# sevagh/Zen

Hardware: AMD Instinct MI355X
Metric: hops/sec (1024-hop HPR, 44.1 kHz mono) (higher is better)
Workload: dtype f32

## Files before the change

zen_amd/csrc/fft_dev.h:

```cpp
#pragma once
#include <type_traits>
#include <hip/hip_runtime.h>

#pragma clang fp contract(off)

namespace zfft {

template <int V>
struct Log2 {
	static constexpr int value = 1 + Log2<V / 2>::value;
};
template <>
struct Log2<1> {
	static constexpr int value = 0;
};

#ifndef ZEN_FFT16K_V
#define ZEN_FFT16K_V 16
#endif

template <int LOG2N>
struct Plan {
	static_assert(LOG2N >= 5 && LOG2N <= 14, "nfft 32..16384");
	static_assert(ZEN_FFT16K_V == 16 || ZEN_FFT16K_V == 32, "16 or 32 values per thread");
// ... 350 lines not shown
			}
		}
#ifdef ZEN_FFT_INPLACE
		if ((FIRST && SYNC_FIRST) || (!FIRST && (!INPL || LAST)))
			frame_sync<TF>();
#else
		if (!FIRST || SYNC_FIRST)
			frame_sync<TF>();
#endif
#pragma unroll
		for (int i = 0; i < NB; ++i) {
			const int b = tf + i * TF;
			const int k = b >> log2J;
			if constexpr (PRE)
				butterfly<R, INV, ZUP, (FIRST && TW::PLAIN)>(v[i], k, sL, LOG2N, twp, PASS, i);
			else
				butterfly<R, INV, ZUP, (FIRST && TW::PLAIN)>(v[i], k, sL, LOG2N, tw, PASS, i);
#pragma unroll
			for (int c = 0; c < R; ++c) {
				const int idx = b + c * (N / R);
				if (LAST) {
					if (!HALF_OUT || c < R / 2) {
						if (active)
							out(idx, v[i][c], c < R / 2, c * NB + i);
					}
				}
#ifdef ZEN_FFT_INPLACE
				else if constexpr (INPL) {
					lds[PL::pad((image_k(k) * R + c) * J + (b & (J - 1)))] = v[i][c];
				}
#endif
				else {
#ifdef ZEN_FFT_FOLD_ADDR
					lds[PL::pad_off(b, c * (N / R))] = v[i][c];
#else
					lds[PL::pad(idx)] = v[i][c];
#endif
				}
			}
		}
		if constexpr (!LAST) {
			frame_sync<TF>();
			PassRunner<LOG2N, PASS + 1, INV, ZU, HALF_OUT, In, Out, SYNC_FIRST, TW>::run(tf, lds, tw, in, out, active);
		}
	}
};

template <int LOG2N, bool INV, bool ZU, bool HALF_OUT, class In, class Out, bool SYNC_FIRST = false>
__device__ __forceinline__ void fft_frame(int tf, float2* __restrict__ lds, const float2* __restrict__ tw,
                                          In& in, Out& out, bool active)
{
	const TwGlobal g{tw};
	PassRunner<LOG2N, 0, INV, ZU, HALF_OUT, In, Out, SYNC_FIRST, TwGlobal>::run(tf, lds, g, in, out, active);
}
template <int LOG2N, bool INV, bool ZU, bool HALF_OUT, class In, class Out, bool SYNC_FIRST = false>
__device__ __forceinline__ void fft_frame(int tf, float2* __restrict__ lds, const TwGlobalPre& tw, In& in, Out& out, bool active)
{
	PassRunner<LOG2N, 0, INV, ZU, HALF_OUT, In, Out, SYNC_FIRST, TwGlobalPre>::run(tf, lds, tw, in, out, active);
}
template <int LOG2N, bool INV, bool ZU, bool HALF_OUT, class In, class Out, bool SYNC_FIRST = false>
__device__ __forceinline__ void fft_frame(int tf, float2* __restrict__ lds, const TwLds& tw, In& in, Out& out, bool active)
{
	PassRunner<LOG2N, 0, INV, ZU, HALF_OUT, In, Out, SYNC_FIRST, TwLds>::run(tf, lds, tw, in, out, active);
}
template <int LOG2N, bool INV, bool ZU, bool HALF_OUT, class In, class Out, bool SYNC_FIRST = false>
__device__ __forceinline__ void fft_frame(int tf, float2* __restrict__ lds, const TwRegs<LOG2N>& tw, In& in, Out& out,
                                          bool active)
{
	PassRunner<LOG2N, 0, INV, ZU, HALF_OUT, In, Out, SYNC_FIRST, TwRegs<LOG2N>>::run(tf, lds, tw, in, out, active);
}

__device__ __forceinline__ double sqrt_of_sum_of_squares(double x)
{
	const double y = __builtin_amdgcn_rsq(x);
	double g = x * y;
	double h = 0.5 * y;
	const double r = __builtin_fma(-h, g, 0.5);
	g = __builtin_fma(g, r, g);
	h = __builtin_fma(h, r, h);
	double d = __builtin_fma(-g, g, x);
	g = __builtin_fma(d, h, g);
	d = __builtin_fma(-g, g, x);
	g = __builtin_fma(d, h, g);
	return (x == 0.0 || x == __builtin_inf()) ? x : g;
}

__device__ __forceinline__ float cabs_exact(float re, float im)
{
	const double r = (double)re, i = (double)im;
	return (float)sqrt_of_sum_of_squares(__builtin_fma(r, r, i * i));
}

}
```

zen_amd/csrc/hpr.hip:

```cpp
#include "common.h"
#include "memguard.h"
#include "filters.h"
#include "hpr_engine.h"
#include "host_pipe.h"

#include <algorithm>
#include <functional>
#include "sse_block.h"
#include "masks.h"
#include "rt_fused.h"
#include "stft.h"

#include <cfloat>
#include <climits>
#include <cmath>
#include <utility>
#include <vector>

using namespace zen_hip_impl;


namespace {
struct ProfScope {
	zen_hip_hpr* e;
// ... 175 lines not shown
	}
	e->tail_sel = 0;
	e->rows_stale = false;
	e->abs_frame = (long long)e->W - 1;
	e->last_frames = 0;
	e->drain[0] = e->drain[1] = e->drain[2] = 0;
	e->ready_valid[0] = e->ready_valid[1] = e->ready_valid[2] = false;
	if (e->d_wide_bar) {
		ZH_HIP(hipStreamSynchronize(e->stream));
		ZH_HIP(hipMemset2DAsync(e->d_wide_bar + 1, sizeof(unsigned) * 4, 0, sizeof(unsigned), S, e->stream));
		*e->wide_fail_host = 0;
	}
	return ZEN_HIP_OK;
}

int ensure_estimates(zen_hip_hpr* e, bool need_h)
{
	const size_t bytes = sizeof(float) * e->n_streams * e->max_hops * e->nfft;
	if (!e->d_P) {
		ZH_HIP(zh_malloc((void**)&e->d_P, bytes));
		ZH_HIP(hipMemsetAsync(e->d_P, 0, bytes, e->stream));
	}
	if (need_h && !e->d_H) {
		ZH_HIP(zh_malloc((void**)&e->d_H, bytes));
		ZH_HIP(hipMemsetAsync(e->d_H, 0, bytes, e->stream));
	}
	return ZEN_HIP_OK;
}

int ensure_rows(zen_hip_hpr* e, int o)
{
	if (e->d_Y[o])
		return ZEN_HIP_OK;
	const size_t bytes = sizeof(float) * e->n_streams * e->max_hops * e->nwin;
	ZH_HIP(zh_malloc((void**)&e->d_Y[o], bytes));
	ZH_HIP(hipMemsetAsync(e->d_Y[o], 0, bytes, e->stream));
	return ZEN_HIP_OK;
}

enum HopKernel { HOP_FUSED = 0, HOP_SSE = 1, HOP_WIDE = 2 };

void fused_args(zen_hip_hpr* e, const float* in, size_t in_stride, size_t M, RtFusedArgs& a)
{
	memset(&a, 0, sizeof(a));
	a.in = in;
	a.in_stride = (long long)in_stride;
	a.tail_prev = e->d_tail[e->tail_sel];
	a.tail_next = e->d_tail[e->tail_sel ^ 1];
	a.window = e->d_window;
	a.tw = e->d_tw;
	a.S = M == 1 ? e->d_S : nullptr;
	a.s_stride = (long long)e->s_stride;
	a.mag = e->d_mag;
	a.keep_mag_rows = (int)e->W - 1;
	a.ring_rows = e->ring_rows;
	a.row0 = e->abs_frame;
	a.hop = (int)e->hop;
	a.n_frames = (int)M;
	a.n_streams = (int)e->n_streams;
	a.prev_frames = (int)e->last_frames;
	a.y_stream_stride = (long long)(e->max_hops * e->nwin);
	for (int o = 0; o < 3; ++o) {
		a.Y[o] = e->d_Y[o];
		e->ready_valid[o] = false;
		if (output_computed(e, o)) {
			a.carry[o] = e->d_carry[o];
			a.out_id[a.n_out++] = o;
			a.ready[o] = e->ready_dev[o];
			e->ready_valid[o] = (M == 1);
		}
	}
	if (M == 1)
		a.seq = ++e->hop_seq;
	a.publish_seq = e->ready_host[0] != nullptr ? (g_opt_publish_release ? 2 : 1) : 0;
	a.beta = e->beta;
	a.beta_h = e->beta - FLT_EPSILON;
	a.cola = e->cola;
	a.soft = e->soft ? 1 : 0;
	a.power = (int)e->beta;
	a.out_h = e->out_h ? 1 : 0;
	a.out_p = e->out_p ? 1 : 0;
	a.thr = ZH_DIAG_OPT(g_opt_mask_divide) ? 0.0 : hard_mask_threshold(e->beta, &a.thr_inclusive);
	a.thr_h = ZH_DIAG_OPT(g_opt_mask_divide) ? 0.0 : hard_mask_threshold(a.beta_h, &a.thr_h_inclusive);
	a.diag = ZH_DIAG_OPT(g_opt_rt_fused_diag);
	a.stamps = e->dbg_stamps;
}

int wide_args(zen_hip_hpr* e, RtFusedArgs& a, hipStream_t stream, bool clear_votes = true)
{
	ZH_TRY(ensure_estimates(e, false));
	if (!e->d_wide_xch) {
		ZH_HIP(zh_malloc((void**)&e->d_wide_xch, sizeof(float2) * e->n_streams * e->nfft));
		ZH_HIP(zh_malloc((void**)&e->d_wide_bar, sizeof(unsigned) * 4 * e->n_streams + 16));
		ZH_HIP(hipMemsetAsync(e->d_wide_bar, 0, sizeof(unsigned) * 4 * e->n_streams + 16, e->stream));
		e->wide_arrivals = 0;
		e->wide_calls = 0;
		void* dev = nullptr;
		ZH_HIP(zh_host_malloc((void**)&e->wide_fail_host, 64, hipHostMallocMapped | hipHostMallocPortable));
		*e->wide_fail_host = 0;
		ZH_HIP(zh_host_device_pointer(&dev, e->wide_fail_host));
		e->wide_fail_dev = (unsigned*)dev;
	}
	if (e->wide_votes_stale && clear_votes) {
		for (size_t st = 0; st < e->n_streams; ++st)
			ZH_HIP(hipMemsetAsync(e->d_wide_bar + 4 * st + 2, 0, 2 * sizeof(unsigned), stream));
		e->wide_votes_stale = false;
	}
	a.wide_fail = e->wide_fail_dev;
	a.P = e->d_P;
	a.p_stream_stride = (long long)(e->max_hops * e->nfft);
	a.xch = e->d_wide_xch;
	a.bar = e->d_wide_bar;
	a.bar_base = e->wide_arrivals;
	a.bar_parity = (int)(e->wide_calls++ & 1u);
	e->wide_arrivals += rt_wide_arrivals(e->log2n, a.n_out);
	return ZEN_HIP_OK;
}

int run_hop_fused(zen_hip_hpr* e, const float* in, size_t in_stride, size_t M, HopKernel kind = HOP_FUSED)
{
	const bool sse = kind == HOP_SSE;
	for (int o = 0; o < 3; ++o)
		if (output_computed(e, o))
			ZH_TRY(ensure_rows(e, o));
	RtFusedArgs a;
	fused_args(e, in, in_stride, M, a);
	if (kind == HOP_WIDE)
		ZH_TRY(wide_args(e, a, e->stream));
	int direct_o = -1;
	for (int o = 0; o < 3; ++o)
		e->direct_done[o] = false;
	bool all_dst = a.n_out > 0;
	for (int i = 0; i < a.n_out; ++i)
		all_dst = all_dst && e->direct_out[a.out_id[i]] != nullptr;
	if (kind == HOP_FUSED && all_dst && !g_opt_no_direct_out && rt_fused_direct_out_available(e->log2n, e->mf, a)) {
		direct_o = a.out_id[0];
		if (!e->d_blk_flag) {
			const size_t bytes = sizeof(unsigned) * e->n_streams * e->max_hops;
			ZH_HIP(zh_malloc((void**)&e->d_blk_flag, bytes));
			ZH_HIP(zh_malloc((void**)&e->d_blk_need, bytes));
			ZH_HIP(hipMemsetAsync(e->d_blk_flag, 0, bytes, e->stream));
			ZH_HIP(hipMemsetAsync(e->d_blk_need, 0, bytes, e->stream));
			e->blk_seq = 0;
		}
		for (int o = 0; o < 3; ++o)
			a.out_direct[o] = e->direct_out[o];
		a.out_direct_stride = e->direct_stride;
		a.direct_on = 1;
		a.blk_flag = e->d_blk_flag;
		a.blk_need = e->d_blk_need;
		e->blk_seq = (e->blk_seq + 1) & 0x0fffffffu;
		if (e->blk_seq == 0)
			e->blk_seq = 1;
		a.blk_seq = e->blk_seq;
	}
	{
		ProfScope ps(e, zen_hip_hpr::K_FUSED);
		if (kind == HOP_WIDE)
			ZH_TRY(launch_rt_wide(e->log2n, e->mf, a, e->stream));
		else if (sse)
			ZH_TRY(launch_rt_sse(e->log2n, a, e->mt, e->mf, (float)e->l_harm + 1.0F, (float)e->l_perc + 1.0F, e->stream));
		else
			ZH_TRY(launch_rt_fused(e->log2n, e->mf, a, e->stream));
	}
	if (direct_o >= 0) {
		ProfScope ps(e, zen_hip_hpr::K_FINALIZE);
// ... 1312 lines not shown
```

zen_amd/csrc/masks.h:

```cpp
#pragma once
#include <hip/hip_runtime.h>

#include <cfloat>
#include <cstring>

#pragma clang fp contract(off)

namespace zen_hip_impl {

struct MaskCfg {
	float beta, beta_h;
	int soft, power, sse, out_h, out_p;
};

__device__ __forceinline__ float powi(float x, int p)
{
	if (p <= 0)
		return 1.0F;
	float r = x;
	for (int i = 1; i < p; ++i)
		r = r * x;
	return r;
}

__device__ __forceinline__ float pmask_value(float h, float p, const MaskCfg& c)
{
	const float EPS = FLT_EPSILON;
	if (c.sse)
		return p * p / (p * p + h * h + EPS);
	if (c.soft) {
		const float xp = powi(p, c.power), yp = powi(h, c.power);
		return xp / (xp + yp + EPS);
	}
	return (float)((p / (h + EPS)) >= c.beta);
}

__device__ __forceinline__ float hmask_value(float h, float p, const MaskCfg& c)
{
	const float EPS = FLT_EPSILON;
	if (c.sse)
		return h * h / (h * h + p * p + EPS);
	if (c.soft) {
		const float xp = powi(h, c.power), yp = powi(p, c.power);
		return xp / (xp + yp + EPS);
	}
	return (float)((h / (p + EPS)) >= c.beta_h);
}

__device__ __forceinline__ float hard_mask_exact(float x, float d, double thr, bool  = false)
{
	const double t = thr * (double)d;
	return (double)x > t ? 1.0F : 0.0F;
}

__device__ __forceinline__ float mask_value(int which, float h, float p, const MaskCfg& c)
{
	if (which == 0)
		return pmask_value(h, p, c);
	if (which == 1)
		return hmask_value(h, p, c);
	const float hm = c.out_h ? hmask_value(h, p, c) : 0.0f;
	const float pm = c.out_p ? pmask_value(h, p, c) : 0.0f;
	return 1 - (hm + pm);
}

struct HardThr {
	double p, h;
	int p_inc, h_inc;
};

__device__ __forceinline__ float pmask_thr(float h, float p, const MaskCfg& c, const HardThr& t)
{
	if (!c.sse && !c.soft && t.p != 0.0)
		return hard_mask_exact(p, h + FLT_EPSILON, t.p, t.p_inc != 0);
	return pmask_value(h, p, c);
}
__device__ __forceinline__ float hmask_thr(float h, float p, const MaskCfg& c, const HardThr& t)
{
	if (!c.sse && !c.soft && t.h != 0.0)
		return hard_mask_exact(h, p + FLT_EPSILON, t.h, t.h_inc != 0);
	return hmask_value(h, p, c);
}
__device__ __forceinline__ float mask_value_thr(int which, float h, float p, const MaskCfg& c, const HardThr& t)
{
	if (which == 0)
		return pmask_thr(h, p, c, t);
	if (which == 1)
		return hmask_thr(h, p, c, t);
	const float hm = c.out_h ? hmask_thr(h, p, c, t) : 0.0f;
	const float pm = c.out_p ? pmask_thr(h, p, c, t) : 0.0f;
	return 1 - (hm + pm);
}

inline double hard_mask_threshold(float beta, int* inclusive)
{
	unsigned u;
	memcpy(&u, &beta, sizeof(u));
	const unsigned expo = (u >> 23) & 0xffu;
	if ((u >> 31) || expo == 0 || expo == 0xffu)
		return 0.0;
	const unsigned up = u - 1;
	float pred;
	memcpy(&pred, &up, sizeof(pred));
	*inclusive = 0;
	const double m = ((double)pred + (double)beta) * 0.5;
	return (u & 1u) == 0 ? m * (1.0 - 0x1p-50) : m;
}
inline HardThr hard_mask_thresholds(float beta, float beta_h, bool divide)
{
	HardThr t{0.0, 0.0, 0, 0};
	if (!divide) {
		t.p = hard_mask_threshold(beta, &t.p_inc);
		t.h = hard_mask_threshold(beta_h, &t.h_inc);
	}
	return t;
}

}
```

zen_amd/csrc/rt_fused.h:

```cpp
#pragma once
#include <hip/hip_runtime.h>

namespace zen_hip_impl {

struct RtFusedArgs {
	const float* in;
	long long in_stride;
	const float* tail_prev;
	float* tail_next;
	const float* window;
	const float2* tw;
	float2* S;
	long long s_stride;
	float* mag;
	int keep_mag_rows;
	long long ring_rows;
	long long row0;
	int hop;
	int n_frames;
	int n_streams;
	int prev_frames;
	float* carry[3];
	float* Y[3];
	long long y_stream_stride;
	float* ready[3];
	unsigned seq;
	int publish_seq;
	int n_out;
	int out_id[3];
	float beta, beta_h, cola;
	int soft, power, out_h, out_p;
	double thr;
	int thr_inclusive;
	double thr_h;
	int thr_h_inclusive;
	float* P;
	long long p_stream_stride;
	float2* xch;
	unsigned* bar;
	unsigned bar_base;
	int bar_parity;
	unsigned* wide_fail;
	float* out_direct[3];
	long long out_direct_stride;
	int direct_on;
	unsigned* blk_flag;
	unsigned* blk_need;
	unsigned blk_seq;
	int diag;
	unsigned long long* stamps;
};

struct ResidentCtl {
	unsigned seq;
	unsigned stop;
	unsigned long long pad;
};
struct ResidentOut {
	unsigned exited;
	unsigned last_seq;
	unsigned hops;
	unsigned pad;
};
int launch_rt_fused_resident(int log2n, int freq_len, const RtFusedArgs& a, const ResidentCtl* ctl, ResidentOut* ro, unsigned seq_start,
                             unsigned long long idle_ticks, unsigned max_hops, hipStream_t stream);
int launch_rt_sse_resident(int log2n, const RtFusedArgs& a, int len_t, int len_f, float fac_h, float fac_p, const ResidentCtl* ctl,
                           ResidentOut* ro, unsigned seq_start, unsigned long long idle_ticks, unsigned max_hops, hipStream_t stream);

#if defined(__HIPCC__)
struct HopOfArgs {
	static constexpr bool KEEP = false;
	const RtFusedArgs& a;
	__device__ __forceinline__ const float* in() const { return a.in; }
	__device__ __forceinline__ unsigned seq() const { return a.seq; }
	__device__ __forceinline__ long long row0() const { return a.row0; }
	__device__ __forceinline__ const float* tail_prev() const { return a.tail_prev; }
	__device__ __forceinline__ float* tail_next() const { return a.tail_next; }
	__device__ __forceinline__ int prev_frames() const { return a.prev_frames; }
};
struct HopVar {
	static constexpr bool KEEP = true;
	mutable float keep_prev[4], keep_carry[4];
	const float* in_;
	unsigned seq_;
	long long row0_;
	const float* tail_prev_;
	float* tail_next_;
	int prev_frames_;
	__device__ __forceinline__ const float* in() const { return in_; }
	__device__ __forceinline__ unsigned seq() const { return seq_; }
	__device__ __forceinline__ long long row0() const { return row0_; }
	__device__ __forceinline__ const float* tail_prev() const { return tail_prev_; }
	__device__ __forceinline__ float* tail_next() const { return tail_next_; }
	__device__ __forceinline__ int prev_frames() const { return prev_frames_; }
};

__device__ __forceinline__ bool resident_next_hop(const ResidentCtl* ctl, unsigned last, unsigned long long idle_ticks, bool leave,
                                                   unsigned* s_cmd, unsigned* sq_out)
{
	if (threadIdx.x == 0) {
		const unsigned long long t0 = __builtin_amdgcn_s_memrealtime();
		unsigned cmd = 2, sq = last;
		for (;;) {
			const unsigned long long w =
			    __hip_atomic_load(reinterpret_cast<const unsigned long long*>(&ctl->seq), __ATOMIC_RELAXED, __HIP_MEMORY_SCOPE_SYSTEM);
			sq = (unsigned)w;
			if (sq != last) {
				cmd = 1;
				break;
			}
			if ((unsigned)(w >> 32) != 0u)
				break;
			if (__builtin_amdgcn_s_memrealtime() - t0 > idle_ticks)
				break;
			__builtin_amdgcn_s_sleep(1);
		}
		s_cmd[0] = leave ? 2u : cmd;
		s_cmd[1] = sq;
// ... 44 lines not shown
```

zen_amd/csrc/rt_fused.hip:

```cpp
#include "common.h"
#include "fft_dev.h"
#include "masks.h"
#include "median47_core.h"
#include "median_net.h"
#include "rt_fused.h"

#include <type_traits>

#pragma clang fp contract(off)

namespace zen_hip_impl {
namespace {

using zfft::Plan;

inline bool hop_lat_takes(int log2n, const RtFusedArgs& a)
{
	return a.n_frames == 1 && log2n <= 12 && !g_opt_no_hop_lat && !a.diag;
}

template <int T>
struct RtImage {
	static constexpr int PAD = T >= 8 ? 4 : 0;
	static constexpr int STRIDE = T + PAD;
	static constexpr int LOG2T = T == 16 ? 4 : (T == 8 ? 3 : 2);
	static __device__ __forceinline__ int addr(int g) { return (g >> LOG2T) * STRIDE + (g & (T - 1)); }
	static constexpr int caddr(int g) { return (g / T) * STRIDE + (g % T); }
	static constexpr int words(int n) { return ((n + T - 1) / T) * STRIDE; }
};

struct Regs {
	float2 S[16];
	float mag[16];
};

template <int LOG2N>
struct FwdIn {
	const float* prev;
	const float* cur;
	const float* window;
	float* tail;
	int hop;
	__device__ __forceinline__ float2 operator()(int idx, int) const
	{
		ZH_CHK(idx < hop ? prev + idx : cur + (idx - hop), 1);
		ZH_CHK(window + idx, 1);
		const float x = idx < hop ? prev[idx] : cur[idx - hop];
		if (tail && idx >= hop) {
			ZH_CHK(tail + (idx - hop), 1);
			tail[idx - hop] = x;
		}
		return make_float2(x * window[idx], 0.0f);
	}
};

struct FwdInPre {
	float x[8], w[8];
	__device__ __forceinline__ float2 operator()(int, int slot) const { return make_float2(x[slot] * w[slot], 0.0f); }
};

template <int T, int TFN>
struct FwdOut {
	Regs* r;
	float2* S;
	float* mag;
	int* img;
	int n, mid_al;
	__device__ __forceinline__ void operator()(int idx, float2 X, bool lower, int slot) const
	{
		r->S[slot] = X;
		if (lower || idx == (n >> 1)) {
			const float m = zfft::cabs_exact(X.x, X.y);
			const int key = __float_as_int(m);
			const int mir = (idx == 0 || idx == (n >> 1)) ? idx : n - idx;
			static_assert(TFN % T == 0, "whole chunks per slot");
			constexpr int CH = (TFN / T) * RtImage<T>::STRIDE;
			const int tfl = idx - slot * TFN;
			const int a0 = RtImage<T>::addr(tfl + mid_al), a1 = RtImage<T>::addr(n - tfl + mid_al);
			img[a0 + slot * CH] = key;
			img[(idx == 0 || idx == (n >> 1)) ? a0 + slot * CH : a1 - slot * CH] = key;
			if (S) {
				ZH_CHK(S + idx, 1);
				S[idx] = X;
			}
			if (mag) {
				ZH_CHK(mag + idx, 1);
				ZH_CHK(mag + mir, 1);
				mag[idx] = m;
				mag[mir] = m;
			}
		}
	}
};

template <int N, int TF, int MID, bool HALF>
struct InvIn {
	const Regs* r;
	const float* P;
	MaskCfg cfg;
	int which;
	__device__ __forceinline__ float2 operator()(int idx, int slot) const
	{
		int pi = idx;
		if (HALF) {
			const int lo = slot * TF, hi = lo + TF - 1;
			if (hi <= N / 2)
				pi = idx;
			else if (lo > N / 2 && hi < N - MID)
				pi = N - idx;
			else
				pi = (idx > N / 2 && idx < N - MID) ? N - idx : idx;
		}
		const float2 z = r->S[slot];
		const float m = mask_value(which, r->mag[slot], P[pi], cfg);
		return make_float2(z.x * m, z.y * m);
	}
};

constexpr int LEAN_PC_WORD = 5184;
constexpr int LEAN_PC_TAIL = 2052;
constexpr int LEAN_EDGE_WORD = LEAN_PC_WORD + LEAN_PC_TAIL + 512 + 4;
template <int N, int TF, int MID, bool HARDP>
struct InvInLean {
	const Regs* r;
	const int* img;
	const float* pc;
	MaskCfg cfg;
	int which;
	double thr;
	bool thr_inclusive;
	__device__ __forceinline__ float2 operator()(int idx, int slot) const
	{
		const int lo = slot * TF, hi = lo + TF - 1;
		int pi;
		if (hi <= N / 2)
			pi = idx;
		else if (lo > N / 2 && hi < N - MID)
			pi = N - idx;
		else
			pi = (idx > N / 2 && idx < N - MID) ? N - idx : (idx > N / 2 ? idx - (N - 512) + LEAN_PC_TAIL : idx);
		const int g = idx + 24;
		const int g0 = g - slot * TF;
		const float mag = __int_as_float(img[(g0 >> 4) * 20 + (g0 & 15) + slot * (TF / 16) * 20]);
		const float2 z = r->S[slot];
		float m;
		if constexpr (HARDP)
			m = hard_mask_exact(pc[pi], mag + FLT_EPSILON, thr, thr_inclusive);
		else
			m = thr != 0.0 ? hard_mask_exact(pc[pi], mag + FLT_EPSILON, thr, thr_inclusive) : mask_value(which, mag, pc[pi], cfg);
		return make_float2(z.x * m, z.y * m);
	}
};

template <int N, int TF, int MID, bool HARDP>
__device__ __forceinline__ unsigned lean_mask_bits(const int* img, const float* pc, int tf, const MaskCfg& cfg, double thr_p,
                                                   double thr_h)
{
	unsigned bits = 0;
#pragma unroll
	for (int slot = 0; slot < 16; ++slot) {
		const int idx = tf + slot * TF, lo = slot * TF, hi = lo + TF - 1;
		int pi;
		if (hi <= N / 2)
			pi = idx;
		else if (lo > N / 2 && hi < N - MID)
			pi = N - idx;
		else
			pi = (idx > N / 2 && idx < N - MID) ? N - idx : (idx > N / 2 ? idx - (N - 512) + LEAN_PC_TAIL : idx);
		const int g = idx + 24;
		const int g0 = tf + 24;
		const float h = __int_as_float(img[(g0 >> 4) * 20 + (g0 & 15) + slot * (TF / 16) * 20]), p = pc[pi];
		(void)g;
		unsigned pm, hm;
		if constexpr (HARDP) {
			pm = cfg.out_p ? (unsigned)(hard_mask_exact(p, h + FLT_EPSILON, thr_p) != 0.0f) : 0u;
			hm = cfg.out_h ? (unsigned)(hard_mask_exact(h, p + FLT_EPSILON, thr_h) != 0.0f) : 0u;
		}
		else {
			const HardThr t{thr_p, thr_h, 0, 0};
			pm = cfg.out_p ? (unsigned)(pmask_thr(h, p, cfg, t) != 0.0f) : 0u;
			hm = cfg.out_h ? (unsigned)(hmask_thr(h, p, cfg, t) != 0.0f) : 0u;
		}
		bits |= (pm | (hm << 1)) << (2 * slot);
	}
	return bits;
}
struct InvInBits {
	const Regs* r;
	unsigned bits;
	int which;
	__device__ __forceinline__ float2 operator()(int, int slot) const
	{
		const float pm = (float)((bits >> (2 * slot)) & 1u), hm = (float)((bits >> (2 * slot + 1)) & 1u);
		const float m = which == 0 ? pm : (which == 1 ? hm : 1 - (hm + pm));
		const float2 z = r->S[slot];
		return make_float2(z.x * m, z.y * m);
	}
};

struct InvOut {
	float* Y;
	float cola;
	float* ready;
	const float* carry;
	int hop;
	__device__ __forceinline__ void operator()(int idx, float2 x, bool, int) const
	{
		const float y = x.x * cola;
		ZH_CHK(Y + idx, 1);
		Y[idx] = y;
		if (ready && idx < hop) {
			ZH_CHK(ready + idx, 1);
			ZH_CHK(carry + idx, 1);
			ready[idx] = carry[idx] + y;
		}
	}
};
__device__ __forceinline__ unsigned xcc_id_of_cu()
{
	unsigned v;
	asm volatile("s_getreg_b32 %0, hwreg(HW_REG_XCC_ID)" : "=s"(v));
	return v & 15u;
}
template <bool KEEP>
struct InvOutRegT {
	float* Y;
	float cola;
	float* ready;
	float cv[4];
	int hop;
	float* next;
	__device__ __forceinline__ void operator()(int idx, float2 x, bool, int slot) const
	{
		const float y = x.x * cola;
		ZH_CHK(Y + idx, 1);
		Y[idx] = y;
		if (ready && idx < hop) {
			ZH_CHK(ready + idx, 1);
			__hip_atomic_store(ready + idx, cv[slot & 3] + y, __ATOMIC_RELAXED, __HIP_MEMORY_SCOPE_SYSTEM);
		}
		if constexpr (KEEP) {
			if (slot >= 4)
				next[slot & 3] = y;
		}
	}
};
using InvOutReg = InvOutRegT<false>;

struct FwdInKeep {
	const float* prev;
	const float* cur;
	const float* window;
	float* next;
	int hop;
	__device__ __forceinline__ float2 operator()(int idx, int slot) const
	{
		float x;
		if (slot < 4) {
			x = prev[slot & 3];
		}
		else {
			ZH_CHK(cur + (idx - hop), 1);
			x = cur[idx - hop];
			next[slot & 3] = x;
		}
		ZH_CHK(window + idx, 1);
		return make_float2(x * window[idx], 0.0f);
	}
};

template <bool LIGHT = false>
__device__ __forceinline__ void publish_ready(unsigned* flag, unsigned seq, int tf, bool release = false)
{
	ZH_CHK(flag, 1);
	if (LIGHT && !release) {
		asm volatile("s_waitcnt vmcnt(0)" ::: "memory");
		__builtin_amdgcn_fence(__ATOMIC_RELEASE, "workgroup");
		__syncthreads();
		if (tf == 0)
			__hip_atomic_store(flag, seq, __ATOMIC_RELAXED, __HIP_MEMORY_SCOPE_SYSTEM);
	}
	else {
		__threadfence_system();
		__syncthreads();
		if (tf == 0)
			__hip_atomic_store(flag, seq, __ATOMIC_RELEASE, __HIP_MEMORY_SCOPE_SYSTEM);
	}
}

template <int LOG2N, int W, int MINB, bool SINGLE, bool LEAN = false, bool HARDP = false, class HV = HopOfArgs>
__device__ __forceinline__ void rt_fused_body(const RtFusedArgs& a, const unsigned bid, const HV& hv, const int tid)
{
	using PL = Plan<LOG2N>;
	constexpr int N = PL::N, TF = PL::TF;
	constexpr int T = znet::outputs_per_thread(W), mid = W / 2;
	static_assert(T >= 4, "needs the 16-byte LDS path");
	using IM = RtImage<T>;
	constexpr int MID_AL = (mid + 3) & ~3, DELTA = MID_AL - mid;
	constexpr int NV = (DELTA + W + T - 1 + 3) / 4, NE = NV * 4;
	constexpr int NCHUNK = N / T, CPT = 16 / T;
	constexpr int IMG_WORDS = IM::words((NCHUNK - 1) * T + NE);
	static_assert(IMG_WORDS * 4 <= PL::LDS_FLOAT2 * 8, "magnitude image must fit in the FFT image");
	constexpr bool BLOCK47 = (W == 47 && LOG2N == 12 && (SINGLE || LEAN));
	static_assert(!LEAN || BLOCK47, "the lean layout is the 47-tap kernel (one output, or several with hard masks)");
	static_assert(!HARDP || LEAN, "the comparison-only mask builds are lean builds");
	static_assert(!LEAN || (LEAN_EDGE_WORD + 256) * 4 <= PL::LDS_FLOAT2 * 8, "lean layout must fit in the frame image");

	extern __shared__ float2 lds[];
	int* img = reinterpret_cast<int*>(lds);
	float* Prow = LEAN ? reinterpret_cast<float*>(img + LEAN_PC_WORD) : reinterpret_cast<float*>(lds + PL::LDS_FLOAT2);

	const int tf = tid, hop = a.hop;
	const int total = a.n_streams * a.n_frames, xq = total >> 3, xr = total & 7, xcd = (int)(bid & 7);
	const int item = xcd * xq + (xcd < xr ? xcd : xr) + (bid >> 3);
	const int s = item / a.n_frames, f = item - s * a.n_frames;
	unsigned long long stamps[6] = {0, 0, 0, 0, 0, 0};
	auto stamp = [&](int k) {
		if constexpr (MINB == 1) {
			if (a.stamps)
				stamps[k] = __builtin_amdgcn_s_memrealtime();
		}
		else {
			if (a.stamps && bid == 0 && tf == 0)
				a.stamps[k] = __builtin_amdgcn_s_memrealtime();
		}
	};
	auto flush_stamps = [&]() {
		if constexpr (MINB == 1) {
			if (a.stamps && bid == 0 && tf == 0) {
#pragma unroll
				for (int k = 0; k < 6; ++k)
					a.stamps[k] = stamps[k];
			}
		}
	};
	stamp(0);
	const float* cur = hv.in() + (long long)s * a.in_stride + (long long)f * hop;

	float cv1[4] = {0.f, 0.f, 0.f, 0.f};
	if constexpr (MINB == 1 && HV::KEEP) {
		static_assert(!HV::KEEP || SINGLE, "one output");
		const int w0 = a.out_id[0];
#pragma unroll
		for (int i = 0; i < 4; ++i) {
			cv1[i] = hv.keep_carry[i];
			ZH_CHK(a.carry[w0] + ((long long)s * hop + tf + i * TF), 1);
			a.carry[w0][(long long)s * hop + tf + i * TF] = cv1[i];
		}
	}
	else if constexpr (MINB == 1) {
		const bool do_carry = hv.prev_frames() > 0 && f == (hv.prev_frames() - 1 < a.n_frames - 1 ? hv.prev_frames() - 1 : a.n_frames - 1);
		float tv[4], sv[3][4];
		if (do_carry) {
#pragma unroll
			for (int o = 0; o < 3; ++o) {
				if (!a.carry[o])
					continue;
				const float* y = a.Y[o] + (long long)s * a.y_stream_stride + (long long)(hv.prev_frames() - 1) * (2 * hop) + hop;
#pragma unroll
				for (int i = 0; i < 4; ++i) {
					ZH_CHK(y + tf + i * TF, 1);
					sv[o][i] = y[tf + i * TF];
				}
			}
		}
		if constexpr (SINGLE) {
			const int w0 = a.out_id[0];
			const float* y = do_carry ? a.Y[w0] + (long long)s * a.y_stream_stride + (long long)(hv.prev_frames() - 1) * (2 * hop) + hop
			                          : a.carry[w0] + (long long)s * hop;
#pragma unroll
			for (int i = 0; i < 4; ++i) {
				ZH_CHK(y + tf + i * TF, 1);
				cv1[i] = y[tf + i * TF];
			}
		}
		if (f == a.n_frames - 1) {
#pragma unroll
			for (int i = 0; i < 4; ++i) {
				ZH_CHK(cur + tf + i * TF, 1);
				tv[i] = cur[tf + i * TF];
			}
		}
		if (do_carry) {
#pragma unroll
			for (int o = 0; o < 3; ++o) {
				if (!a.carry[o])
					continue;
#pragma unroll
				for (int i = 0; i < 4; ++i) {
					ZH_CHK(a.carry[o] + ((long long)s * hop + tf + i * TF), 1);
					a.carry[o][(long long)s * hop + tf + i * TF] = sv[o][i];
				}
			}
// ... 66 lines not shown
				ZH_CHK(a.blk_need + item, 1);
				a.blk_need[item] = 1u;
			}
			if (xi >= DIRECT_BACK) {
				dh = item - DIRECT_BACK;
				const int hs = dh / a.n_frames, hf = dh - hs * a.n_frames;
				unsigned v0 = 0, v1 = 0;
				if (hf > 0) {
					ZH_CHK(a.blk_flag + dh - 1, 2);
					v0 = __hip_atomic_load(a.blk_flag + dh - 1, __ATOMIC_RELAXED, __HIP_MEMORY_SCOPE_AGENT);
					v1 = __hip_atomic_load(a.blk_flag + dh, __ATOMIC_RELAXED, __HIP_MEMORY_SCOPE_AGENT);
				}
				preload_inputs();
				if (hf > 0) {
					const unsigned want = (a.blk_seq << 4) | xcc_id_of_cu();
					dcomb = v0 == want && v1 == want;
				}
				if (dcomb && SINGLE) {
					const int which = a.out_id[0];
					const unsigned* row = reinterpret_cast<const unsigned*>(a.Y[which] + (long long)hs * a.y_stream_stride
					                                                        + (long long)hf * (2 * hop));
#pragma unroll
					for (int i = 0; i < 4; ++i) {
						ZH_CHK(row - hop + tf + i * TF, 1);
						ZH_CHK(row + tf + i * TF, 1);
						dv[i] = __hip_atomic_load(row - hop + tf + i * TF, __ATOMIC_RELAXED, __HIP_MEMORY_SCOPE_AGENT);
						dv[4 + i] = __hip_atomic_load(row + tf + i * TF, __ATOMIC_RELAXED, __HIP_MEMORY_SCOPE_AGENT);
					}
				}
				else if (dcomb) {
					unsigned dm[3][8];
#pragma unroll
					for (int oi = 0; oi < 3; ++oi) {
						if (oi < a.n_out) {
							const unsigned* row = reinterpret_cast<const unsigned*>(a.Y[a.out_id[oi]] + (long long)hs * a.y_stream_stride
							                                                        + (long long)hf * (2 * hop));
#pragma unroll
							for (int i = 0; i < 4; ++i) {
								ZH_CHK(row - hop + tf + i * TF, 1);
								ZH_CHK(row + tf + i * TF, 1);
								dm[oi][i] = __hip_atomic_load(row - hop + tf + i * TF, __ATOMIC_RELAXED, __HIP_MEMORY_SCOPE_AGENT);
								dm[oi][4 + i] = __hip_atomic_load(row + tf + i * TF, __ATOMIC_RELAXED, __HIP_MEMORY_SCOPE_AGENT);
							}
						}
					}
#pragma unroll
					for (int oi = 0; oi < 3; ++oi) {
						if (oi < a.n_out) {
							float* o = a.out_direct[a.out_id[oi]] + (long long)hs * a.out_direct_stride + (long long)hf * hop;
#pragma unroll
							for (int i = 0; i < 4; ++i) {
								ZH_CHK(o + tf + i * TF, 1);
								o[tf + i * TF] = __uint_as_float(dm[oi][i]) + __uint_as_float(dm[oi][4 + i]);
							}
						}
					}
				}
				else {
					ZH_CHK(a.blk_need + dh, 1);
					a.blk_need[dh] = 1u;
				}
			}
		}
	}
	constexpr bool TWC = (MINB == 1);
	zfft::TwRegs<LOG2N> twr;
	if constexpr (TWC)
		twr.fill(tf, a.tw);
	Regs r;
	{
		FwdIn<LOG2N> in;
		in.prev = f > 0 ? cur - hop : hv.tail_prev() + (long long)s * hop;
		in.cur = cur;
		in.window = a.window;
		in.tail = (MINB == 1 || f != a.n_frames - 1) ? nullptr : hv.tail_next() + (long long)s * hop;
		in.hop = hop;
		const long long row = ((hv.row0() + f) % a.ring_rows) + (long long)s * a.ring_rows;
		FwdOut<T, TF> out;
		out.r = &r;
		out.S = a.S ? a.S + row * a.s_stride : nullptr;
		out.mag = (a.S || f >= a.n_frames - a.keep_mag_rows) ? a.mag + row * N : nullptr;
		out.img = img;
		out.n = N;
		out.mid_al = MID_AL;
		if constexpr (DIRECT) {
			if (!preloaded)
				preload_inputs();
			if (in.tail) {
#pragma unroll
				for (int m = 4; m < 8; ++m) {
					ZH_CHK(in.tail + ((m - 4) * TF + tf), 1);
					in.tail[(m - 4) * TF + tf] = pre.x[m];
				}
			}
			zfft::fft_frame<LOG2N, false, true, false>(tf, lds, a.tw, pre, out, true);
		}
		else if constexpr (TWC && HV::KEEP) {
			float nx[4];
			FwdInKeep ink{hv.keep_prev, cur, a.window, nx, hop};
			zfft::fft_frame<LOG2N, false, true, false>(tf, lds, twr, ink, out, true);
#pragma unroll
			for (int i = 0; i < 4; ++i) {
				ZH_CHK(hv.tail_next() + ((long long)s * hop + tf + i * TF), 1);
				hv.tail_next()[(long long)s * hop + tf + i * TF] = nx[i];
				hv.keep_prev[i] = nx[i];
			}
		}
		else if constexpr (TWC)
			zfft::fft_frame<LOG2N, false, true, false>(tf, lds, twr, in, out, true);
		else
			zfft::fft_frame<LOG2N, false, true, false>(tf, lds, a.tw, in, out, true);
	}
	__syncthreads();
	if constexpr (DIRECT && SINGLE) {
		if (dcomb) {
			const int hs = dh / a.n_frames, hf = dh - hs * a.n_frames;
			float* o = a.out_direct[a.out_id[0]] + (long long)hs * a.out_direct_stride + (long long)hf * hop;
#pragma unroll
			for (int i = 0; i < 4; ++i) {
				ZH_CHK(o + tf + i * TF, 1);
				o[tf + i * TF] = __uint_as_float(dv[i]) + __uint_as_float(dv[4 + i]);
			}
		}
	}
	stamp(2);
	{
		const int v0 = img[IM::addr(MID_AL)], v1 = img[IM::addr(N - 1 + MID_AL)];
		for (int g = tf; g < MID_AL; g += TF)
			img[IM::addr(g)] = v0;
		for (int g = N + MID_AL + tf; g < (NCHUNK - 1) * T + NE; g += TF)
			img[IM::addr(g)] = v1;
	}
	__syncthreads();

	if (a.diag == 1) {
		for (int k = tf; k < (LEAN ? 2048 : N); k += TF)
			Prow[k] = __int_as_float(img[IM::addr(k + MID_AL)]);
	}
	else if constexpr (BLOCK47) {
		static_assert(IM::STRIDE == zm47::RSTR && MID_AL == 24 && TF == 256, "image layout of median47_core.h");
		int(*edge)[64] = LEAN ? reinterpret_cast<int(*)[64]>(img + LEAN_EDGE_WORD) : reinterpret_cast<int(*)[64]>(Prow + N);
		const int lane = tf & 63, wave = __builtin_amdgcn_readfirstlane(tf >> 6);
		const int blk = wave < 2 ? tf : (lane < 32 ? 128 + lane : 192 + lane);
		zm47::Pieces pc;
		if (wave < 3)
			zm47::m47_sort_and_publish(img, edge, blk, lane, wave, tf == 0, blk == 255, pc);
		__syncthreads();
		if (wave < 3) {
			int out[16];
			zm47::m47_select(img, edge, blk, wave, pc, out);
			if constexpr (LEAN) {
				const int at = blk >= 224 ? LEAN_PC_TAIL + (blk - 224) * 16 : blk * 16;
				if (blk <= 127 || blk >= 224) {
#pragma unroll
					for (int v = 0; v < 4; ++v)
						*reinterpret_cast<int4*>(&Prow[at + 4 * v]) =
						    make_int4(out[4 * v], out[4 * v + 1], out[4 * v + 2], out[4 * v + 3]);
				}
				else if (blk == 128) {
					*reinterpret_cast<int4*>(&Prow[at]) = make_int4(out[0], out[1], out[2], out[3]);
				}
			}
			else {
#pragma unroll
				for (int v = 0; v < 4; ++v)
					*reinterpret_cast<int4*>(&Prow[blk * 16 + 4 * v]) =
					    make_int4(out[4 * v], out[4 * v + 1], out[4 * v + 2], out[4 * v + 3]);
			}
		}
	}
	else {
#pragma unroll
	for (int ci = 0; ci < CPT; ++ci) {
		const int ch = tf * CPT + ci;
		int ld[NE], e[W + T - 1], out[T];
		const int* mine = &img[ch * IM::STRIDE];
#pragma unroll
		for (int v = 0; v < NV; ++v) {
			const int4 q = *reinterpret_cast<const int4*>(mine + IM::caddr(4 * v));
			ld[4 * v] = q.x;
			ld[4 * v + 1] = q.y;
			ld[4 * v + 2] = q.z;
			ld[4 * v + 3] = q.w;
		}
#pragma unroll
		for (int q = 0; q < W + T - 1; ++q)
			e[q] = ld[q + DELTA];
		znet::medians<W, T, W + T - 1>(e, out);
#pragma unroll
		for (int v = 0; v < T / 4; ++v)
			*reinterpret_cast<int4*>(&Prow[ch * T + 4 * v]) =
			    make_int4(out[4 * v], out[4 * v + 1], out[4 * v + 2], out[4 * v + 3]);
	}
	}
	__syncthreads();
	stamp(3);
	if constexpr (LEAN && !SINGLE) {
		if (a.diag == 2)
			return;
		const MaskCfg cfg{a.beta, a.beta_h, 0, a.power, 0, a.out_h, a.out_p};
		const unsigned bits = lean_mask_bits<N, TF, mid, HARDP>(img, Prow, tf, cfg, a.thr, a.thr_h);
		__syncthreads();
		for (int oi = 0; oi < a.n_out; ++oi) {
			const int which = a.out_id[oi];
			InvInBits in{&r, bits, which};
			OutT out;
			out.Y = a.Y[which] + (long long)s * a.y_stream_stride + (long long)f * (2 * hop);
			out.cola = a.cola;
			out.ready = (a.n_frames == 1 && a.ready[which]) ? a.ready[which] + (long long)s * hop : nullptr;
			if constexpr (MINB == 1) {
				pick_carry(which, out.cv);
			}
			else {
				out.carry = a.carry[which] + (long long)s * hop;
			}
			out.hop = hop;
			int tf_o = tf;
			int tw_off = 0;
			asm volatile("" : "+v"(tf_o));
			asm volatile("" : "+s"(tw_off));
			const float2* tw_o = a.tw + tw_off;
			if constexpr (TWC)
				zfft::fft_frame<LOG2N, true, false, true>(tf_o, lds, twr, in, out, true);
			else
				zfft::fft_frame<LOG2N, true, false, true>(tf_o, lds, tw_o, in, out, true);
			if (out.ready && a.publish_seq)
				publish_ready<MINB == 1>(reinterpret_cast<unsigned*>(out.ready + hop), hv.seq(), tf, a.publish_seq == 2);
			__syncthreads();
		}
		if constexpr (DIRECT) {
			if (a.direct_on) {
				asm volatile("s_waitcnt vmcnt(0)" ::: "memory");
				__builtin_amdgcn_fence(__ATOMIC_RELEASE, "workgroup");
				__syncthreads();
				if (tf == 0)
					__hip_atomic_store(a.blk_flag + item, (a.blk_seq << 4) | xcc_id_of_cu(), __ATOMIC_RELAXED, __HIP_MEMORY_SCOPE_AGENT);
			}
		}
		return;
	}
	else if constexpr (LEAN) {
		if (a.diag == 2)
			return;
		InvInLean<N, TF, mid, HARDP> in;
		in.r = &r;
		in.img = img;
		in.pc = Prow;
		in.cfg = MaskCfg{a.beta, a.beta_h, a.soft, a.power, 0, a.out_h, a.out_p};
		in.which = a.out_id[0];
		in.thr = (in.which == 0 && !a.soft) ? a.thr : 0.0;
		in.thr_inclusive = a.thr_inclusive != 0;
		if constexpr (DIRECT && SINGLE) {
			InvOut out;
			out.Y = a.Y[in.which] + (long long)s * a.y_stream_stride + (long long)f * (2 * hop);
			out.cola = a.cola;
			out.ready = nullptr;
			out.carry = nullptr;
			out.hop = hop;
			zfft::fft_frame<LOG2N, true, false, true, InvInLean<N, TF, mid, HARDP>, InvOut, true>(tf, lds, a.tw, in, out, true);
			if (a.direct_on) {
				asm volatile("s_waitcnt vmcnt(0)" ::: "memory");
				__builtin_amdgcn_fence(__ATOMIC_RELEASE, "workgroup");
				__syncthreads();
				if (tf == 0)
					__hip_atomic_store(a.blk_flag + item, (a.blk_seq << 4) | xcc_id_of_cu(), __ATOMIC_RELAXED, __HIP_MEMORY_SCOPE_AGENT);
			}
			return;
		}
		OutT out;
		out.Y = a.Y[in.which] + (long long)s * a.y_stream_stride + (long long)f * (2 * hop);
		out.cola = a.cola;
		out.ready = (a.n_frames == 1 && a.ready[in.which]) ? a.ready[in.which] + (long long)s * hop : nullptr;
		if constexpr (MINB == 1) {
			pick_carry(in.which, out.cv);
			out.next = cnext;
		}
		else {
			out.carry = a.carry[in.which] + (long long)s * hop;
		}
		out.hop = hop;
		if constexpr (TWC)
			zfft::fft_frame<LOG2N, true, false, true, InvInLean<N, TF, mid, HARDP>, OutT, true>(tf, lds, twr, in, out, true);
		else
			zfft::fft_frame<LOG2N, true, false, true, InvInLean<N, TF, mid, HARDP>, OutT, true>(tf, lds, a.tw, in, out, true);
		if constexpr (HV::KEEP) {
#pragma unroll
			for (int i = 0; i < 4; ++i)
				hv.keep_carry[i] = cnext[i];
		}
		if (out.ready && a.publish_seq)
			publish_ready<MINB == 1>(reinterpret_cast<unsigned*>(out.ready + hop), hv.seq(), tf, a.publish_seq == 2);
		if constexpr (MINB == 1) {
			stamp(4);
			stamp(5);
			flush_stamps();
		}
		return;
	}
#pragma unroll
	for (int slot = 0; slot < 16; ++slot)
		r.mag[slot] = __int_as_float(img[IM::addr(tf + slot * TF + MID_AL)]);
	__syncthreads();

	auto synth = [&](int which) {
		InvIn<N, TF, mid, BLOCK47> in;
		in.r = &r;
		in.P = Prow;
		in.cfg = MaskCfg{a.beta, a.beta_h, a.soft, a.power, 0, a.out_h, a.out_p};
		in.which = which;
		OutT out;
		out.Y = a.Y[which] + (long long)s * a.y_stream_stride + (long long)f * (2 * hop);
		out.cola = a.cola;
		out.ready = (a.n_frames == 1 && a.ready[which]) ? a.ready[which] + (long long)s * hop : nullptr;
		if constexpr (MINB == 1) {
			pick_carry(which, out.cv);
			out.next = cnext;
		}
		else {
			out.carry = a.carry[which] + (long long)s * hop;
		}
		out.hop = hop;
		if constexpr (TWC)
			zfft::fft_frame<LOG2N, true, false, true>(tf, lds, twr, in, out, true);
		else
			zfft::fft_frame<LOG2N, true, false, true>(tf, lds, a.tw, in, out, true);
		if constexpr (HV::KEEP) {
#pragma unroll
			for (int i = 0; i < 4; ++i)
				hv.keep_carry[i] = cnext[i];
		}
		if (out.ready && a.publish_seq)
			publish_ready<MINB == 1>(reinterpret_cast<unsigned*>(out.ready + hop), hv.seq(), tf, a.publish_seq == 2);
	};
	if (a.diag == 2) {
		if (tf == 0)
			a.Y[a.out_id[0]][(long long)s * a.y_stream_stride + (long long)f * (2 * hop)] = Prow[tf] + r.mag[3] + r.S[5].x;
		return;
	}
	stamp(4);
	if constexpr (SINGLE) {
		synth(a.out_id[0]);
		stamp(5);
		flush_stamps();
	}
	else {
		for (int oi = 0; oi < a.n_out; ++oi) {
			synth(a.out_id[oi]);
			__syncthreads();
		}
	}
}

template <int LOG2N, int W, int MINB, bool SINGLE, bool LEAN = false, bool HARDP = false>
__global__ __launch_bounds__(Plan<LOG2N>::TF, MINB) void rt_fused_kernel(RtFusedArgs a)
{
	rt_fused_body<LOG2N, W, MINB, SINGLE, LEAN, HARDP>(a, blockIdx.x, HopOfArgs{a}, (int)threadIdx.x);
}

template <int LOG2N, int W, int MINB, bool SINGLE, bool LEAN = false, bool HARDP = false>
int launch_k(const RtFusedArgs& a, hipStream_t stream)
{
	using PL = Plan<LOG2N>;
	const size_t lds = LEAN ? sizeof(float2) * PL::LDS_FLOAT2
	                        : sizeof(float2) * PL::LDS_FLOAT2 + sizeof(float) * PL::N + (W == 47 && LOG2N == 12 && SINGLE ? 1024 : 0);
	auto kern = rt_fused_kernel<LOG2N, W, MINB, SINGLE, LEAN, HARDP>;
	if (lds > 64 * 1024)
		ZH_HIP(hipFuncSetAttribute((const void*)kern, hipFuncAttributeMaxDynamicSharedMemorySize, (int)lds));
// ... 228 lines not shown
```

Before: 53.39 million.

## Use single-precision power-of-two mask test, shifted median image, and rank-based median tail

```diff
diff --git a/zen_amd/csrc/fft_dev.h b/zen_amd/csrc/fft_dev.h
--- a/zen_amd/csrc/fft_dev.h
+++ b/zen_amd/csrc/fft_dev.h
@@ -456,13 +456,22 @@
 	g = __builtin_fma(d, h, g);
 	d = __builtin_fma(-g, g, x);
 	g = __builtin_fma(d, h, g);
+#if defined(ZEN_CABS_GUARD64)
 	return (x == 0.0 || x == __builtin_inf()) ? x : g;
+#else
+	return g;
+#endif
 }
 
 __device__ __forceinline__ float cabs_exact(float re, float im)
 {
 	const double r = (double)re, i = (double)im;
-	return (float)sqrt_of_sum_of_squares(__builtin_fma(r, r, i * i));
-}
-
-}
+	const float m = (float)sqrt_of_sum_of_squares(__builtin_fma(r, r, i * i));
+#if defined(ZEN_CABS_GUARD64)
+	return m;
+#else
+	return __builtin_fminf(m, __builtin_fabsf(re) + __builtin_fabsf(im));
+#endif
+}
+
+}
diff --git a/zen_amd/csrc/hpr.hip b/zen_amd/csrc/hpr.hip
--- a/zen_amd/csrc/hpr.hip
+++ b/zen_amd/csrc/hpr.hip
@@ -281,6 +281,7 @@
 	a.out_p = e->out_p ? 1 : 0;
 	a.thr = ZH_DIAG_OPT(g_opt_mask_divide) ? 0.0 : hard_mask_threshold(e->beta, &a.thr_inclusive);
 	a.thr_h = ZH_DIAG_OPT(g_opt_mask_divide) ? 0.0 : hard_mask_threshold(a.beta_h, &a.thr_h_inclusive);
+	a.nbeta_pow2 = a.thr != 0.0 ? hard_mask_pow2_beta(e->beta) : 0.0F;
 	a.diag = ZH_DIAG_OPT(g_opt_rt_fused_diag);
 	a.stamps = e->dbg_stamps;
 }
diff --git a/zen_amd/csrc/masks.h b/zen_amd/csrc/masks.h
--- a/zen_amd/csrc/masks.h
+++ b/zen_amd/csrc/masks.h
@@ -53,6 +53,11 @@
 	return (double)x > t ? 1.0F : 0.0F;
 }
 
+__device__ __forceinline__ float hard_mask_pow2(float x, float d, float nbeta)
+{
+	return __builtin_fmaf(nbeta, d, x) >= 0.0F ? 1.0F : 0.0F;
+}
+
 __device__ __forceinline__ float mask_value(int which, float h, float p, const MaskCfg& c)
 {
 	if (which == 0)
@@ -106,6 +111,15 @@
 	const double m = ((double)pred + (double)beta) * 0.5;
 	return (u & 1u) == 0 ? m * (1.0 - 0x1p-50) : m;
 }
+inline float hard_mask_pow2_beta(float beta)
+{
+	unsigned u;
+	memcpy(&u, &beta, sizeof(u));
+	const unsigned expo = (u >> 23) & 0xffu;
+	if ((u >> 31) || (u & 0x7fffffu) || expo < 127u - 64u || expo > 127u + 64u)
+		return 0.0F;
+	return -beta;
+}
 inline HardThr hard_mask_thresholds(float beta, float beta_h, bool divide)
 {
 	HardThr t{0.0, 0.0, 0, 0};
diff --git a/zen_amd/csrc/median47_tail.h b/zen_amd/csrc/median47_tail.h
--- /dev/null
+++ b/zen_amd/csrc/median47_tail.h
@@ -0,0 +1,28 @@
+#pragma once
+#include <hip/hip_runtime.h>
+
+namespace zm47 {
+
+__device__ __forceinline__ int m47_tail_by_rank(int u, int lane)
+{
+	const int x1 = __builtin_amdgcn_readlane(u, 1);
+	const int a_lt = x1 < u ? 1 : 0, a_le = x1 <= u ? 1 : 0;
+	int lt = lane < 2 ? 64 : 0, le = 0;
+	int res = lane == 0 ? u : x1;
+#pragma unroll
+	for (int i = 2; i <= 46; ++i) {
+		const int b = __builtin_amdgcn_readlane(u, i);
+		lt += b < u ? 1 : 0;
+		le += b <= u ? 1 : 0;
+		if (i >= 25) {
+			const int k = i - 23, c = 25 - k;
+			const bool q = lane <= i && lt + c * a_lt <= 23 && le + c * a_le > 23;
+			const unsigned long long m = __builtin_amdgcn_ballot_w64(q);
+			const int src = m != 0ull ? (int)__builtin_ctzll(m) : 1;
+			res = lane == k ? __builtin_amdgcn_readlane(u, src) : res;
+		}
+	}
+	return res;
+}
+
+}
diff --git a/zen_amd/csrc/rt_fused.h b/zen_amd/csrc/rt_fused.h
--- a/zen_amd/csrc/rt_fused.h
+++ b/zen_amd/csrc/rt_fused.h
@@ -34,6 +34,7 @@
 	int thr_inclusive;
 	double thr_h;
 	int thr_h_inclusive;
+	float nbeta_pow2;
 	float* P;
 	long long p_stream_stride;
 	float2* xch;
diff --git a/zen_amd/csrc/rt_fused.hip b/zen_amd/csrc/rt_fused.hip
--- a/zen_amd/csrc/rt_fused.hip
+++ b/zen_amd/csrc/rt_fused.hip
@@ -2,6 +2,7 @@
 #include "fft_dev.h"
 #include "masks.h"
 #include "median47_core.h"
+#include "median47_tail.h"
 #include "median_net.h"
 #include "rt_fused.h"
 
@@ -120,8 +121,19 @@
 constexpr int LEAN_PC_WORD = 5184;
 constexpr int LEAN_PC_TAIL = 2052;
 constexpr int LEAN_EDGE_WORD = LEAN_PC_WORD + LEAN_PC_TAIL + 512 + 4;
-template <int N, int TF, int MID, bool HARDP>
+#if defined(ZEN_NO_LEAN_SHIFT)
+constexpr bool LEAN_SHIFT_ON = false;
+#else
+constexpr bool LEAN_SHIFT_ON = true;
+#endif
+#if defined(ZEN_NO_POW2_MASK)
+constexpr bool LEAN_POW2_ON = false;
+#else
+constexpr bool LEAN_POW2_ON = true;
+#endif
+template <int N, int TF, int MID, bool HARDP, bool POW2 = false, int SH = 0>
 struct InvInLean {
+	static_assert(!POW2 || HARDP, "the single-precision comparison is a HARDP variant");
 	const Regs* r;
 	const int* img;
 	const float* pc;
@@ -129,6 +141,7 @@
 	int which;
 	double thr;
 	bool thr_inclusive;
+	float nbeta;
 	__device__ __forceinline__ float2 operator()(int idx, int slot) const
 	{
 		const int lo = slot * TF, hi = lo + TF - 1;
@@ -139,12 +152,14 @@
 			pi = N - idx;
 		else
 			pi = (idx > N / 2 && idx < N - MID) ? N - idx : (idx > N / 2 ? idx - (N - 512) + LEAN_PC_TAIL : idx);
-		const int g = idx + 24;
+		const int g = idx + 24 - SH;
 		const int g0 = g - slot * TF;
 		const float mag = __int_as_float(img[(g0 >> 4) * 20 + (g0 & 15) + slot * (TF / 16) * 20]);
 		const float2 z = r->S[slot];
 		float m;
-		if constexpr (HARDP)
+		if constexpr (POW2)
+			m = hard_mask_pow2(pc[pi], mag + FLT_EPSILON, nbeta);
+		else if constexpr (HARDP)
 			m = hard_mask_exact(pc[pi], mag + FLT_EPSILON, thr, thr_inclusive);
 		else
 			m = thr != 0.0 ? hard_mask_exact(pc[pi], mag + FLT_EPSILON, thr, thr_inclusive) : mask_value(which, mag, pc[pi], cfg);
@@ -152,9 +167,9 @@
 	}
 };
 
-template <int N, int TF, int MID, bool HARDP>
+template <int N, int TF, int MID, bool HARDP, bool POW2 = false, int SH = 0>
 __device__ __forceinline__ unsigned lean_mask_bits(const int* img, const float* pc, int tf, const MaskCfg& cfg, double thr_p,
-                                                   double thr_h)
+                                                   double thr_h, float nbeta = 0.0f)
 {
 	unsigned bits = 0;
 #pragma unroll
@@ -167,13 +182,16 @@
 			pi = N - idx;
 		else
 			pi = (idx > N / 2 && idx < N - MID) ? N - idx : (idx > N / 2 ? idx - (N - 512) + LEAN_PC_TAIL : idx);
-		const int g = idx + 24;
-		const int g0 = tf + 24;
+		const int g = idx + 24 - SH;
+		const int g0 = tf + 24 - SH;
 		const float h = __int_as_float(img[(g0 >> 4) * 20 + (g0 & 15) + slot * (TF / 16) * 20]), p = pc[pi];
 		(void)g;
 		unsigned pm, hm;
 		if constexpr (HARDP) {
-			pm = cfg.out_p ? (unsigned)(hard_mask_exact(p, h + FLT_EPSILON, thr_p) != 0.0f) : 0u;
+			if constexpr (POW2)
+				pm = cfg.out_p ? (unsigned)(hard_mask_pow2(p, h + FLT_EPSILON, nbeta) != 0.0f) : 0u;
+			else
+				pm = cfg.out_p ? (unsigned)(hard_mask_exact(p, h + FLT_EPSILON, thr_p) != 0.0f) : 0u;
 			hm = cfg.out_h ? (unsigned)(hard_mask_exact(h, p + FLT_EPSILON, thr_h) != 0.0f) : 0u;
 		}
 		else {
@@ -309,6 +327,9 @@
 	extern __shared__ float2 lds[];
 	int* img = reinterpret_cast<int*>(lds);
 	float* Prow = LEAN ? reinterpret_cast<float*>(img + LEAN_PC_WORD) : reinterpret_cast<float*>(lds + PL::LDS_FLOAT2);
+	constexpr int SH = (LEAN && MINB != 1 && LEAN_SHIFT_ON) ? 1 : 0;
+	constexpr bool POW2_OK = HARDP && MINB != 1 && LEAN_POW2_ON;
+	float* pcv = Prow + 3 * SH;
 
 	const int tf = tid, hop = a.hop;
 	const int total = a.n_streams * a.n_frames, xq = total >> 3, xr = total & 7, xcd = (int)(bid & 7);
@@ -541,7 +562,7 @@
 		out.mag = (a.S || f >= a.n_frames - a.keep_mag_rows) ? a.mag + row * N : nullptr;
 		out.img = img;
 		out.n = N;
-		out.mid_al = MID_AL;
+		out.mid_al = MID_AL - SH;
 		if constexpr (DIRECT) {
 			if (!preloaded)
 				preload_inputs();
@@ -583,7 +604,12 @@
 		}
 	}
 	stamp(2);
-	{
+	if constexpr (SH) {
+		const int v0 = img[IM::addr(MID_AL - SH)];
+		if (tf < MID_AL - SH)
+			img[IM::addr(tf)] = v0;
+	}
+	else {
 		const int v0 = img[IM::addr(MID_AL)], v1 = img[IM::addr(N - 1 + MID_AL)];
 		for (int g = tf; g < MID_AL; g += TF)
 			img[IM::addr(g)] = v0;
@@ -594,7 +620,30 @@
 
 	if (a.diag == 1) {
 		for (int k = tf; k < (LEAN ? 2048 : N); k += TF)
-			Prow[k] = __int_as_float(img[IM::addr(k + MID_AL)]);
+			pcv[k] = __int_as_float(img[IM::addr(k + MID_AL - SH)]);
+	}
+	else if constexpr (BLOCK47 && SH != 0) {
+		static_assert(IM::STRIDE == zm47::RSTR && MID_AL == 24 && TF == 256, "image layout of median47_core.h");
+		int(*edge)[64] = reinterpret_cast<int(*)[64]>(img + LEAN_EDGE_WORD);
+		const int lane = tf & 63, wave = __builtin_amdgcn_readfirstlane(tf >> 6);
+		const int blk = wave < 2 ? tf : 128 + lane;
+		zm47::Pieces pc;
+		if (wave < 3) {
+			zm47::m47_sort_and_publish(img, edge, blk, lane, wave, tf == 0, false, pc);
+		}
+		else {
+			const int res = zm47::m47_tail_by_rank(img[IM::addr(lane + MID_AL - SH)], lane);
+			if (lane <= mid)
+				pcv[lane == 0 ? 0 : LEAN_PC_TAIL + 512 - lane] = __int_as_float(res);
+		}
+		__syncthreads();
+		if (wave < 2) {
+			int out[16];
+			zm47::m47_select(img, edge, blk, wave, pc, out);
+#pragma unroll
+			for (int v = 0; v < 4; ++v)
+				*reinterpret_cast<int4*>(&Prow[blk * 16 + 4 + 4 * v]) = make_int4(out[4 * v], out[4 * v + 1], out[4 * v + 2], out[4 * v + 3]);
+		}
 	}
 	else if constexpr (BLOCK47) {
 		static_assert(IM::STRIDE == zm47::RSTR && MID_AL == 24 && TF == 256, "image layout of median47_core.h");
@@ -658,7 +707,13 @@
 		if (a.diag == 2)
 			return;
 		const MaskCfg cfg{a.beta, a.beta_h, 0, a.power, 0, a.out_h, a.out_p};
-		const unsigned bits = lean_mask_bits<N, TF, mid, HARDP>(img, Prow, tf, cfg, a.thr, a.thr_h);
+		unsigned bits;
+		if constexpr (POW2_OK) {
+			bits = a.nbeta_pow2 != 0.0f ? lean_mask_bits<N, TF, mid, HARDP, true, SH>(img, pcv, tf, cfg, a.thr, a.thr_h, a.nbeta_pow2)
+			                            : lean_mask_bits<N, TF, mid, HARDP, false, SH>(img, pcv, tf, cfg, a.thr, a.thr_h);
+		}
+		else
+			bits = lean_mask_bits<N, TF, mid, HARDP, false, SH>(img, pcv, tf, cfg, a.thr, a.thr_h);
 		__syncthreads();
 		for (int oi = 0; oi < a.n_out; ++oi) {
 			const int which = a.out_id[oi];
@@ -701,14 +756,19 @@
 	else if constexpr (LEAN) {
 		if (a.diag == 2)
 			return;
-		InvInLean<N, TF, mid, HARDP> in;
-		in.r = &r;
-		in.img = img;
-		in.pc = Prow;
-		in.cfg = MaskCfg{a.beta, a.beta_h, a.soft, a.power, 0, a.out_h, a.out_p};
-		in.which = a.out_id[0];
-		in.thr = (in.which == 0 && !a.soft) ? a.thr : 0.0;
-		in.thr_inclusive = a.thr_inclusive != 0;
+		using InL = InvInLean<N, TF, mid, HARDP, false, SH>;
+		InL in;
+		auto fill_in = [&](auto& q) {
+			q.r = &r;
+			q.img = img;
+			q.pc = pcv;
+			q.cfg = MaskCfg{a.beta, a.beta_h, a.soft, a.power, 0, a.out_h, a.out_p};
+			q.which = a.out_id[0];
+			q.thr = (q.which == 0 && !a.soft) ? a.thr : 0.0;
+			q.thr_inclusive = a.thr_inclusive != 0;
+			q.nbeta = a.nbeta_pow2;
+		};
+		fill_in(in);
 		if constexpr (DIRECT && SINGLE) {
 			InvOut out;
 			out.Y = a.Y[in.which] + (long long)s * a.y_stream_stride + (long long)f * (2 * hop);
@@ -716,7 +776,14 @@
 			out.ready = nullptr;
 			out.carry = nullptr;
 			out.hop = hop;
-			zfft::fft_frame<LOG2N, true, false, true, InvInLean<N, TF, mid, HARDP>, InvOut, true>(tf, lds, a.tw, in, out, true);
+			if (POW2_OK && a.nbeta_pow2 != 0.0f) {
+				using InP = InvInLean<N, TF, mid, HARDP, POW2_OK, SH>;
+				InP inp;
+				fill_in(inp);
+				zfft::fft_frame<LOG2N, true, false, true, InP, InvOut, true>(tf, lds, a.tw, inp, out, true);
+			}
+			else
+				zfft::fft_frame<LOG2N, true, false, true, InL, InvOut, true>(tf, lds, a.tw, in, out, true);
 			if (a.direct_on) {
 				asm volatile("s_waitcnt vmcnt(0)" ::: "memory");
 				__builtin_amdgcn_fence(__ATOMIC_RELEASE, "workgroup");
@@ -739,9 +806,9 @@
 		}
 		out.hop = hop;
 		if constexpr (TWC)
-			zfft::fft_frame<LOG2N, true, false, true, InvInLean<N, TF, mid, HARDP>, OutT, true>(tf, lds, twr, in, out, true);
+			zfft::fft_frame<LOG2N, true, false, true, InL, OutT, true>(tf, lds, twr, in, out, true);
 		else
-			zfft::fft_frame<LOG2N, true, false, true, InvInLean<N, TF, mid, HARDP>, OutT, true>(tf, lds, a.tw, in, out, true);
+			zfft::fft_frame<LOG2N, true, false, true, InL, OutT, true>(tf, lds, a.tw, in, out, true);
 		if constexpr (HV::KEEP) {
 #pragma unroll
 			for (int i = 0; i < 4; ++i)
```

New measurement: 50.93 million. -4.6%, worse.
